# nanoporetech/medaka

Hardware: NVIDIA H100
Metric: pileup positions/sec (consensus inference) (higher is better)
Workload: dtype f32

## Files before the change

include/medaka_b200.h:

```cpp
#ifndef MEDAKA_B200_H
#define MEDAKA_B200_H

#include <stddef.h>
#include <stdint.h>

#ifdef __cplusplus
extern "C" {
#endif

#define MDK_OK 0
#define MDK_ERR_ARG -1
#define MDK_ERR_CUDA -2
#define MDK_ERR_STATE -3
#define MDK_ERR_UNSUPPORTED -4
#define MDK_ERR_NOMEM -5

#define MDK_PREC_TC 0
#define MDK_PREC_FP32 1

#define MDK_REC_AUTO 0
#define MDK_REC_ONE_TILE 1
#define MDK_REC_PINGPONG 2

#define MDK_NORM_TOTAL 0
#define MDK_NORM_FWD_REV 1
#define MDK_NORM_NONE 2

typedef struct mdk_engine mdk_engine;
typedef struct mdk_bam mdk_bam;
typedef struct mdk_bam_batch mdk_bam_batch;

typedef struct mdk_model_desc {
    int32_t num_features;
    int32_t gru_size;
    int32_t n_layers;
    int32_t bidirectional;
    int32_t num_classes;
} mdk_model_desc;

typedef struct mdk_timings {
    float h2d_ms;
    float inproj0_ms;
    float rec0_ms;
    float inproj1_ms;
    float rec1_ms;
    float head_ms;
    float d2h_ms;
    float total_ms;
    int32_t launches;
} mdk_timings;

const char *mdk_plp_bases(void);
size_t mdk_featlen(void);
size_t mdk_fwd_del(void);
size_t mdk_rev_del(void);

const char *mdk_last_error(void);
const char *mdk_version(void);
int mdk_device_count(int *count);
int mdk_device_info(int device, int *sm_arch, int *sm_count, size_t *total_mem);

int mdk_host_alloc(size_t bytes, void **out);
int mdk_host_free(void *p);
int mdk_dev_alloc(int device, size_t bytes, void **out);
int mdk_dev_free(int device, void *p);
int mdk_memcpy_h2d(int device, void *dst_dev, const void *src_host, size_t bytes);
int mdk_memcpy_d2h(int device, void *dst_host, const void *src_dev, size_t bytes);
int mdk_dev_memset(int device, void *dst_dev, int value, size_t bytes);
int mdk_device_synchronize(int device);

int mdk_engine_create(int device, const mdk_model_desc *desc, mdk_engine **out);
int mdk_engine_destroy(mdk_engine *e);
int mdk_engine_load_gru(mdk_engine *e, int layer, int direction, const float *w_ih,
                        const float *w_hh, const float *b_ih, const float *b_hh);
int mdk_engine_load_linear(mdk_engine *e, const float *w, const float *b);
// ... 94 lines not shown
                  mdk_bam_batch **out);
int64_t mdk_bam_batch_size(mdk_bam_batch *x);
int mdk_bam_batch_arrays(mdk_bam_batch *x, const int32_t **pos, const uint16_t **flag, const uint8_t **mapq,
                         const int32_t **l_seq, const uint32_t **cigar, const int64_t **cigar_off,
                         const uint8_t **seq, const int64_t **seq_off, const uint8_t **aux, const int64_t **aux_off,
                         const char **names, const int64_t **name_off);
int mdk_bam_batch_qual(mdk_bam_batch *x, const uint8_t **qual, const int64_t **qual_off);
int mdk_bam_batch_free(mdk_bam_batch *x);

int mdk_annotate(int device, int64_t n_rec, const int32_t *pos, const uint16_t *flag, const uint8_t *mapq,
                 const uint8_t *dtype, const uint32_t *cigar, const int64_t *cigar_off, const uint8_t *seq,
                 const int64_t *seq_off, const uint8_t *contig, int32_t contig_start, int32_t contig_n,
                 int32_t contig_len, int64_t n_var, const int32_t *var_pos, const int32_t *var_ref_len,
                 const int64_t *hap_off, const int64_t *allele_off, const uint8_t *alleles, int32_t pad,
                 int32_t min_mapq, int32_t dpsp, const int8_t *score, int32_t gap_open, int32_t gap_extend,
                 int64_t *dp_out, int64_t *sr_out, int64_t *ar_out, int64_t *sc_out, int64_t *stats_out,
                 float *kernel_ms);

int mdk_decode_consensus(int device, const float *probs, int64_t n, uint8_t *labels_out,
                         uint8_t *quals_out);
int mdk_decode_consensus_dev(int device, const float *probs_dev, int64_t n,
                             uint8_t *labels_out_dev, uint8_t *quals_out_dev);
int mdk_decode_consensus_f64(int device, const double *probs, int64_t n, uint8_t *labels_out,
                             uint8_t *quals_out);

int mdk_stitch_consensus(int device, const float *const *seg_probs, const int64_t *seg_rows, int64_t n_seg,
                         uint8_t *seq_out, uint8_t *qual_out, int64_t *seg_out_off);
int mdk_stitch_consensus_dev(int device, const float *probs_dev, int64_t n_rows, const int64_t *seg_base,
                             int64_t n_seg, uint8_t *seq_out_dev, uint8_t *qual_out_dev, int64_t *seg_out_off);
int mdk_stitch_labels_dev(int device, const uint8_t *labels_dev, const uint8_t *quals_dev,
                          const int64_t *seg_start, const int64_t *seg_rows, int64_t n_seg,
                          uint8_t *seq_out, uint8_t *qual_out, int64_t *seg_out_off);
int mdk_variant_join_cuts(int device, const uint8_t *const *seg_calls, const int64_t *seg_rows, int64_t n_seg,
                          int64_t *cut_out);
int mdk_decode_variants_dev(int device, const uint8_t *const *seg_calls, const float *const *seg_pred_q,
                            const float *const *seg_ref_q, const int64_t *seg_rows, int64_t n_seg,
                            const int64_t *sample_seg, int64_t n_samples, int64_t max_runs, int64_t *run_sample,
                            int64_t *run_start, int64_t *run_len, float *run_pred_q, float *run_ref_q,
                            int64_t max_run_cols, uint8_t *run_pred, float *run_col_pred_q, float *run_col_ref_q,
                            float *ref_q_out, int64_t *n_runs_out, int64_t *n_run_cols_out);

int mdk_variant_columns(int device, const int64_t *minor, const uint8_t *reference,
                        const uint8_t *prediction, uint8_t *out, int64_t len);

int mdk_decode_variants(int device, const float *probs, const int64_t *minor, const uint8_t *ref_code, int64_t n,
                        uint8_t *pred_out, uint8_t *is_var_out, float *pred_q_out, float *ref_q_out, int64_t max_runs,
                        int64_t *run_start, int64_t *run_len, float *run_pred_q, float *run_ref_q,
                        int64_t *n_runs_out);

int mdk_selftest_umma(int device, const float *A, const float *B, float *D, int N, int K,
                      int variant);

int mdk_debug_timeline(mdk_engine *e, int n_last, float *out);
int mdk_debug_read_plog(mdk_engine *e, float *out_host, int64_t n_floats);
int mdk_rl_debug_read(mdk_rl_engine *e, int which, float *out_host, int64_t n_floats);

typedef struct mdk_trainer mdk_trainer;

#define MDK_OPT_RMSPROP 0
#define MDK_OPT_ADAM 1
#define MDK_OPT_NADAM 2
#define MDK_OPT_SGD 3

typedef struct mdk_optim_desc {
    int32_t kind;
    float alpha, beta1, beta2, eps, weight_decay, momentum, dampening, momentum_decay;
    int32_t nesterov;
} mdk_optim_desc;

typedef struct mdk_train_stats {
    double loss;
    int64_t n_correct;
    int64_t n_positions;
    float grad_norm;
    int32_t skipped;
} mdk_train_stats;

int mdk_trainer_create(int device, const mdk_model_desc *desc, mdk_trainer **out);
int mdk_trainer_destroy(mdk_trainer *tr);
int mdk_trainer_load_gru(mdk_trainer *tr, int layer, int direction, const float *w_ih, const float *w_hh,
                         const float *b_ih, const float *b_hh);
int mdk_trainer_load_linear(mdk_trainer *tr, const float *w, const float *b);
int mdk_trainer_set_optimizer(mdk_trainer *tr, const mdk_optim_desc *opt);
int mdk_trainer_step(mdk_trainer *tr, const float *feats, const int32_t *labels, int64_t B, int64_t T, float lr,
                     float max_norm, mdk_train_stats *stats);
int mdk_trainer_eval(mdk_trainer *tr, const float *feats, const int32_t *labels, int64_t B, int64_t T, float *probs,
                     float *logits, mdk_train_stats *stats);
int mdk_trainer_num_params(mdk_trainer *tr, int64_t *n);
int mdk_trainer_read_params(mdk_trainer *tr, float *out_host, int64_t n);
int mdk_trainer_read_grads(mdk_trainer *tr, float *out_host, int64_t n);
int mdk_trainer_workspace_bytes(const mdk_model_desc *desc, int64_t B, int64_t T, size_t *bytes, size_t *budget);
int mdk_trainer_stage_ms(mdk_trainer *tr, float *ms);
int mdk_trainer_set_bptt_windows(mdk_trainer *tr, int nb);

typedef struct mdk_rl_trainer mdk_rl_trainer;

int mdk_rl_trainer_create(int device, int32_t lstm_size, int32_t cnn_size, int32_t use_dwells, int32_t num_classes,
                          mdk_rl_trainer **out);
int mdk_rl_trainer_destroy(mdk_rl_trainer *tr);
int mdk_rl_trainer_load(mdk_rl_trainer *tr, const char *name, const float *data, int64_t n);
int mdk_rl_trainer_set_optimizer(mdk_rl_trainer *tr, const mdk_optim_desc *opt);
int mdk_rl_trainer_step(mdk_rl_trainer *tr, const int8_t *x, const int32_t *labels, int64_t B, int64_t P, int64_t D,
                        int64_t F, float lr, float max_norm, mdk_train_stats *stats);
int mdk_rl_trainer_eval(mdk_rl_trainer *tr, const int8_t *x, const int32_t *labels, int64_t B, int64_t P, int64_t D,
                        int64_t F, float *probs, float *logits, mdk_train_stats *stats);
int mdk_rl_trainer_num_params(mdk_rl_trainer *tr, int64_t *n);
// ... 15 lines not shown
```

medaka_b200/csrc/api.cu:

```cuda
#include <algorithm>
#include <cstdlib>
#include <cstring>
#include <new>

#include "common.cuh"
#include "gru_pack.cuh"

namespace mdk {

static thread_local std::string g_last_error;

void set_error(const std::string &msg) { g_last_error = msg; }

int cuda_fail(cudaError_t err, const char *what, const char *file, int line) {
    char buf[512];
    snprintf(buf, sizeof(buf), "CUDA error %d (%s) at %s:%d: %s", (int)err, cudaGetErrorString(err), file, line, what);
    g_last_error = buf;
    if (err == cudaErrorMemoryAllocation) {
        cudaGetLastError();
        return MDK_ERR_NOMEM;
    }
    return MDK_ERR_CUDA;
}

// ... 126 lines not shown
}

static int ensure_quals(mdk_lane &ln) {
    if (ln.cap_quals >= ln.cap_io && ln.d_quals) return MDK_OK;
    dev_free(ln.d_quals);
    ln.cap_quals = 0;
    int rc;
    if ((rc = dev_alloc(&ln.d_quals, (size_t)ln.cap_io))) return rc;
    ln.cap_quals = ln.cap_io;
    return MDK_OK;
}

static int ensure_var(mdk_lane &ln) {
    if (ln.cap_var >= ln.cap_io && ln.d_ref) return MDK_OK;
    dev_free(ln.d_ref); dev_free(ln.d_calls); dev_free(ln.d_pred_q); dev_free(ln.d_ref_q);
    ln.cap_var = 0;
    int rc;
    if ((rc = dev_alloc(&ln.d_ref, (size_t)ln.cap_io))) return rc;
    if ((rc = dev_alloc(&ln.d_calls, (size_t)ln.cap_io))) return rc;
    if ((rc = dev_alloc(&ln.d_pred_q, (size_t)ln.cap_io))) return rc;
    if ((rc = dev_alloc(&ln.d_ref_q, (size_t)ln.cap_io))) return rc;
    ln.cap_var = ln.cap_io;
    return MDK_OK;
}

static int run_forward256(mdk_engine *e, mdk_ws &ws, const float *feats_dev, int64_t B, int64_t T, float *probs_dev,
                          float *logits_dev, uint8_t *labels_dev, uint8_t *quals_dev, const HeadVariant *var) {
    int rc;
    if ((rc = ensure_h1(ws, H2_256))) return rc;
    const int64_t P = B * T;
    cudaStream_t s = ws.stream, s1 = ws.l1_stream;
    const bool tc = e->precision == MDK_PREC_TC;
    const LayerWeights &l0 = e->layer[0], &l1 = e->layer[1];
    float *h0 = static_cast<float *>(ws.h0);
    MDK_CUDA(cudaStreamWaitEvent(s, ws.l1_done, 0));
    MDK_CUDA(cudaEventRecord(e->ev[1], s));
    MDK_CUDA(launch_inproj0(feats_dev, l0.w_in_packed, l0.bias_gi, ws.gi, P, e->desc.num_features,
                            T, tc ? 1 : 0, s, H256));
    MDK_CUDA(cudaEventRecord(e->ev[2], s));
    if (tc) MDK_CUDA(launch_rec256_tc(ws.gi, l0.w_hh_tm, l0.b_hn_tc, h0, B, T, s));
    else MDK_CUDA(launch_rec_fp32(ws.gi, l0.w_hh_t, l0.b_hn, h0, B, T, s, H256));
    MDK_CUDA(cudaEventRecord(e->ev[3], s));
    if (tc) MDK_CUDA(launch_gemm256_tc(h0, l1.w_in_tc, l1.bias_gi_tc, ws.gi, tiled_rows(B, T), s));
    else MDK_CUDA(launch_gemm_fp32(h0, l1.w_in_packed, l1.bias_gi, ws.gi, P, H2_256, GI256_COLS, s));
    MDK_CUDA(cudaEventRecord(e->ev[4], s));
    MDK_CUDA(cudaStreamWaitEvent(s1, e->ev[4], 0));
    if (tc) MDK_CUDA(launch_rec256_tc(ws.gi, l1.w_hh_tm, l1.b_hn_tc, ws.h1, B, T, s1));
    else MDK_CUDA(launch_rec_fp32(ws.gi, l1.w_hh_t, l1.b_hn, ws.h1, B, T, s1, H256));
    MDK_CUDA(cudaEventRecord(e->ev[5], s1));
    MDK_CUDA(cudaEventRecord(ws.l1_done, s1));
    MDK_CUDA(launch_head(ws.h1, e->lin_w, e->lin_b, B, T, tc ? 1 : 0, probs_dev, logits_dev, labels_dev, s1, quals_dev,
                         var, H2_256));
    MDK_CUDA(cudaEventRecord(e->ev[6], s1));
    e->launches += 5;
    e->last.launches = 5;
    ws.last_fused_head = false;
    ws.last_B = B; ws.last_T = T; ws.last_precision = e->precision;
    e->last_ws = (int)(&ws - e->ws);
    return MDK_OK;
}

static int run_forward(mdk_engine *e, mdk_ws &ws, const float *feats_dev, int64_t B, int64_t T, float *probs_dev,
                       float *logits_dev, uint8_t *labels_dev, uint8_t *quals_dev, const HeadVariant *var) {
    int rc;
    if ((rc = prepare_weights(e))) return rc;
    if ((rc = ensure_workspace(e, ws, B, T))) return rc;
    if (e->desc.gru_size == H256)
        return run_forward256(e, ws, feats_dev, B, T, probs_dev, logits_dev, labels_dev, quals_dev, var);
    const int64_t P = B * T;
    cudaStream_t s = ws.stream, s1 = ws.l1_stream;
    const bool tc = e->precision == MDK_PREC_TC;
    int launches = 0;
    const bool fuse_x = tc && e->layer[0].w_x_tm != nullptr;
    const int64_t tiles = (B + WT - 1) / WT;
    const int tiles_per_cta = e->rec_mode == MDK_REC_PINGPONG ? 2
                            : e->rec_mode == MDK_REC_ONE_TILE ? 1
                            : fuse_x || tiles * NDIR > (int64_t)e->sm_count ? 2 : 1;
    const bool fuse_head = tc && !e->keep_act;
    if (!fuse_head && (rc = ensure_h1(ws, H2))) return rc;
    if (!fuse_x) MDK_CUDA(cudaStreamWaitEvent(s, ws.l1_done, 0));
    MDK_CUDA(cudaEventRecord(e->ev[1], s));
    if (!fuse_x) {
        MDK_CUDA(launch_inproj0(feats_dev, e->layer[0].w_in_packed, e->layer[0].bias_gi, ws.gi, P,
                                e->desc.num_features, T, tc ? 1 : 0, s));
        launches++;
    }
    MDK_CUDA(cudaEventRecord(e->ev[2], s));
    if (tc) {
        const RecX fx{feats_dev, e->layer[0].w_x_tm, e->layer[0].bias_gi_tc, e->desc.num_features};
        MDK_CUDA(launch_rec_tc(ws.gi, fuse_x ? &fx : nullptr, e->layer[0].w_hh_tm, e->layer[0].b_hn_tc, tiles_per_cta,
                               OUT_TILES, ws.h0, nullptr, B, T, s));
    } else {
        MDK_CUDA(launch_rec_fp32(ws.gi, e->layer[0].w_hh_t, e->layer[0].b_hn, (float *)ws.h0, B, T, s));
    }
    launches++;
    if (fuse_x) MDK_CUDA(cudaStreamWaitEvent(s, ws.l1_done, 0));
    MDK_CUDA(cudaEventRecord(e->ev[3], s));
    if (tc) MDK_CUDA(launch_gemm_tc(ws.h0, e->layer[1].w_in_tc, e->layer[1].bias_gi_tc, ws.gi, tiled_rows(B, T), e->sm_count, s));
    else MDK_CUDA(launch_gemm_fp32((const float *)ws.h0, e->layer[1].w_in_packed, e->layer[1].bias_gi, ws.gi, P, H2, GI_COLS, s));
    launches++;
    MDK_CUDA(cudaEventRecord(e->ev[4], s));
    MDK_CUDA(cudaStreamWaitEvent(s1, e->ev[4], 0));
    if (tc) {
        MDK_CUDA(launch_rec_tc(ws.gi, nullptr, e->layer[1].w_hh_tm, e->layer[1].b_hn_tc, tiles_per_cta,
                               fuse_head ? OUT_LOGITS : OUT_ROWS, fuse_head ? (void *)ws.plog : ws.h1, e->lin_w, B, T, s1));
    } else {
        MDK_CUDA(launch_rec_fp32(ws.gi, e->layer[1].w_hh_t, e->layer[1].b_hn, ws.h1, B, T, s1));
    }
    launches++;
    MDK_CUDA(cudaEventRecord(e->ev[5], s1));
    MDK_CUDA(cudaEventRecord(ws.l1_done, s1));
    if (fuse_head) MDK_CUDA(launch_head_plog(ws.plog, e->lin_b, B, T, probs_dev, logits_dev, labels_dev, s1, quals_dev, var));
    else MDK_CUDA(launch_head(ws.h1, e->lin_w, e->lin_b, B, T, tc ? 1 : 0, probs_dev, logits_dev, labels_dev, s1, quals_dev,
                              var));
    launches++;
    MDK_CUDA(cudaEventRecord(e->ev[6], s1));
    e->launches += launches;
    e->last.launches = launches;
    ws.last_fused_head = fuse_head;
    ws.last_B = B; ws.last_T = T; ws.last_precision = e->precision;
    e->last_ws = (int)(&ws - e->ws);
    return MDK_OK;
}

static int acquire_lane(mdk_engine *e, int64_t P, int *out) {
    int idx;
    if (P > mdk_engine::SMALL_POS) {
        idx = e->next_big;
        e->next_big = (e->next_big + 1) % mdk_engine::BIG_LANES;
    } else {
        idx = mdk_engine::BIG_LANES + e->next_small;
        e->next_small = (e->next_small + 1) % mdk_engine::SMALL_LANES;
    }
    mdk_lane &ln = e->lane[idx];
    if (ln.busy) {
        MDK_CUDA(cudaEventSynchronize(ln.ev_out));
        ln.busy = false;
    }
    *out = idx;
    return MDK_OK;
}

struct GruCall {
    mdk_engine *e;
    const float *feats = nullptr;
    int64_t B = 0, T = 0;
    const uint8_t *ref = nullptr;

    int open(int64_t windows) {
        const int rc = acquire_lane(e, B * T, &e->open_lane);
        return rc ? rc : ensure_io(e, e->lane[e->open_lane], windows, T);
    }
    int64_t capacity(int64_t len) {
        const mdk_lane &ln = e->lane[e->open_lane];
        return std::min(ln.cap_io / len, ln.cap_feats / (len * e->desc.num_features));
    }
    int stage(int64_t first, int64_t n, int64_t at) {
        const size_t w = (size_t)T * e->desc.num_features;
        mdk_lane &ln = e->lane[e->open_lane];
        MDK_CUDA(cudaMemcpyAsync(ln.d_feats + at * w, feats + first * w, n * w * sizeof(float), cudaMemcpyDefault,
                                 e->copy_in));
        if (ref) {
            int rc;
            if ((rc = ensure_var(ln))) return rc;
            MDK_CUDA(cudaMemcpyAsync(ln.d_ref + at * T, ref + first * T, n * T, cudaMemcpyDefault, e->copy_in));
        }
        return MDK_OK;
    }
    int launch() {
// ... 362 lines not shown

static void stage_times(cudaEvent_t *ev, mdk_timings *t) {
    t->h2d_ms = ev_ms(ev[0], ev[1]);
    t->inproj0_ms = ev_ms(ev[1], ev[2]);
    t->rec0_ms = ev_ms(ev[2], ev[3]);
    t->inproj1_ms = ev_ms(ev[3], ev[4]);
    t->rec1_ms = ev_ms(ev[4], ev[5]);
    t->head_ms = ev_ms(ev[5], ev[6]);
    t->d2h_ms = ev_ms(ev[6], ev[7]);
    t->total_ms = ev_ms(ev[0], ev[7]);
}

int mdk_engine_last_timings(mdk_engine *e, mdk_timings *out) { return mdk_engine_mean_timings(e, 1, out); }

int mdk_engine_mean_timings(mdk_engine *e, int n_last, mdk_timings *out) {
    MDK_REQUIRE(e && out, MDK_ERR_ARG, "NULL argument");
    MDK_REQUIRE(n_last >= 1 && n_last <= mdk_engine::EV_RING, MDK_ERR_ARG, "mean_timings: n_last out of range");
    MDK_CUDA(cudaSetDevice(e->device));
    int rc = launch_group(e);
    if (rc) return rc;
    MDK_REQUIRE(e->fwd_count >= 1, MDK_ERR_STATE, "mean_timings: no forward recorded");
    n_last = (int)std::min<int64_t>(n_last, e->fwd_count);
    for (auto &ws : e->ws) MDK_CUDA(ws_sync(ws));
    mdk_timings acc{};
    for (int i = 0; i < n_last; ++i) {
        mdk_timings t{};
        stage_times(e->evr[(e->fwd_count - 1 - i) % mdk_engine::EV_RING], &t);
        acc.h2d_ms += t.h2d_ms; acc.inproj0_ms += t.inproj0_ms; acc.rec0_ms += t.rec0_ms;
        acc.inproj1_ms += t.inproj1_ms; acc.rec1_ms += t.rec1_ms; acc.head_ms += t.head_ms;
        acc.d2h_ms += t.d2h_ms; acc.total_ms += t.total_ms;
    }
    const float inv = 1.0f / (float)n_last;
    acc.h2d_ms *= inv; acc.inproj0_ms *= inv; acc.rec0_ms *= inv; acc.inproj1_ms *= inv; acc.rec1_ms *= inv;
    acc.head_ms *= inv; acc.d2h_ms *= inv; acc.total_ms *= inv;
    acc.launches = e->last.launches;
    *out = acc;
    return MDK_OK;
}

int mdk_debug_timeline(mdk_engine *e, int n_last, float *out) {
    MDK_REQUIRE(e && out, MDK_ERR_ARG, "NULL argument");
    MDK_CUDA(cudaSetDevice(e->device));
    int rc = launch_group(e);
    if (rc) return rc;
    MDK_REQUIRE(n_last >= 1 && n_last <= mdk_engine::EV_RING && e->fwd_count >= n_last, MDK_ERR_ARG, "timeline: bad n_last");
    for (auto &ws : e->ws) MDK_CUDA(ws_sync(ws));
    for (int i = 0; i < n_last; ++i) {
        cudaEvent_t *ev = e->evr[(e->fwd_count - n_last + i) % mdk_engine::EV_RING];
        for (int k = 0; k < 8; ++k) MDK_CUDA(cudaEventElapsedTime(out + i * 8 + k, e->ev_timer[0], ev[k]));
    }
    return MDK_OK;
}

int mdk_engine_timer_start(mdk_engine *e) {
    MDK_REQUIRE(e, MDK_ERR_ARG, "engine is NULL");
    MDK_CUDA(cudaSetDevice(e->device));
    int rc = mdk_engine_sync(e);
    if (rc) return rc;
    MDK_CUDA(cudaEventRecord(e->ev_timer[0], e->stream));
    for (int i = 0; i < mdk_engine::N_WS; ++i) {
        if (i) MDK_CUDA(cudaStreamWaitEvent(e->ws[i].stream, e->ev_timer[0], 0));
        MDK_CUDA(cudaStreamWaitEvent(e->ws[i].l1_stream, e->ev_timer[0], 0));
    }
    MDK_CUDA(cudaStreamWaitEvent(e->copy_in, e->ev_timer[0], 0));
    return MDK_OK;
}
int mdk_engine_timer_stop(mdk_engine *e, float *elapsed_ms) {
    MDK_REQUIRE(e && elapsed_ms, MDK_ERR_ARG, "NULL argument");
    MDK_CUDA(cudaSetDevice(e->device));
    int rc = launch_group(e);
    if (rc) return rc;
    for (int i = 0; i < mdk_engine::N_WS; ++i) {
        if (i) {
            MDK_CUDA(cudaEventRecord(e->ev_join, e->ws[i].stream));
            MDK_CUDA(cudaStreamWaitEvent(e->stream, e->ev_join, 0));
        }
        MDK_CUDA(cudaEventRecord(e->ev_join, e->ws[i].l1_stream));
        MDK_CUDA(cudaStreamWaitEvent(e->stream, e->ev_join, 0));
    }
    MDK_CUDA(cudaEventRecord(e->ev_join, e->copy_out.stream));
    MDK_CUDA(cudaStreamWaitEvent(e->stream, e->ev_join, 0));
    MDK_CUDA(cudaEventRecord(e->ev_timer[1], e->stream));
    MDK_CUDA(cudaEventSynchronize(e->ev_timer[1]));
    MDK_CUDA(cudaEventElapsedTime(elapsed_ms, e->ev_timer[0], e->ev_timer[1]));
    return MDK_OK;
}

int mdk_engine_read_activation(mdk_engine *e, int which, float *out_host, int64_t n_floats) {
    MDK_REQUIRE(e, MDK_ERR_ARG, "engine is NULL");
    return mdk_engine_read_activation_windows(e, which, 0, e->ws[e->last_ws].last_B, out_host, n_floats);
}

int mdk_engine_read_activation_windows(mdk_engine *e, int which, int64_t first, int64_t count, float *out_host,
                                       int64_t n_floats) {
    MDK_REQUIRE(e && out_host, MDK_ERR_ARG, "NULL argument");
    MDK_REQUIRE(which == 0 || which == 1, MDK_ERR_ARG, "read_activation: which must be 0 or 1");
    mdk_ws &ln = e->ws[e->last_ws];
    MDK_REQUIRE(ln.last_B > 0 && ln.last_T > 0, MDK_ERR_STATE, "read_activation: no forward recorded");
    MDK_REQUIRE(first >= 0 && count > 0 && first + count <= ln.last_B, MDK_ERR_ARG,
                "read_activation: windows first .. first + count - 1 must lie in the last forward's B windows");
    const int width = 2 * e->desc.gru_size;
    MDK_REQUIRE(n_floats == count * ln.last_T * width, MDK_ERR_ARG, "read_activation: size must be count*T*2*gru_size");
    MDK_REQUIRE(!(which == 1 && ln.last_fused_head), MDK_ERR_STATE,
                "read_activation(1): the last forward fused the head into layer 1 (h1 never reached HBM); call "
                "mdk_engine_keep_activations(e, 1) before the forward");
    MDK_CUDA(cudaSetDevice(e->device));
// ... 54 lines not shown
```

medaka_b200/csrc/common.cuh:

```cuda
#pragma once
#include <cuda_runtime.h>
#include <cuda_fp16.h>

#include <cstdint>
#include <cstdio>
#include <string>
#include <vector>

#include "../../include/medaka_b200.h"
#include "packing.h"

namespace mdk {

constexpr int H = 128;
constexpr int G3 = 3 * H;
constexpr int NDIR = 2;
constexpr int GI_COLS = NDIR * G3;
constexpr int H2 = NDIR * H;
constexpr int NCLS = 5;
constexpr int H256 = 256;
constexpr int G3_256 = 3 * H256;
constexpr int GI256_COLS = NDIR * G3_256;
constexpr int H2_256 = NDIR * H256;

// ... 174 lines not shown
}

struct mdk_ws {
    cudaStream_t stream = nullptr;
    cudaStream_t l1_stream = nullptr;
    cudaEvent_t l1_done = nullptr;
    int64_t cap_pos = 0;
    float *gi = nullptr;
    void *h0 = nullptr;
    float *h1 = nullptr;
    int64_t cap_h1 = 0;
    float *plog = nullptr;
    int64_t last_B = 0, last_T = 0;
    int last_precision = -1;
    bool last_fused_head = false;
};

struct mdk_lane {
    mdk_ws *ws = nullptr;
    int64_t cap_io = 0;
    int64_t cap_quals = 0;
    int64_t cap_var = 0;
    int64_t cap_feats = 0;
    float *d_feats = nullptr, *d_probs = nullptr, *d_logits = nullptr;
    uint8_t *d_labels = nullptr, *d_quals = nullptr;
    uint8_t *d_ref = nullptr, *d_calls = nullptr;
    float *d_pred_q = nullptr, *d_ref_q = nullptr;
    cudaEvent_t ev_in = nullptr, ev_out = nullptr;
    bool busy = false;
};

struct mdk_engine {
    int device = 0;
    mdk_model_desc desc{};
    int precision = MDK_PREC_TC;
    int sm_count = 132;
    int rec_mode = MDK_REC_AUTO;
    int64_t wave256 = 0;
    static constexpr int BIG_WS = 1, BIG_LANES = 4, SMALL_LANES = 14;
    static constexpr int N_LANES = BIG_LANES + SMALL_LANES, N_WS = BIG_WS + SMALL_LANES;
    static constexpr int64_t SMALL_POS = 1 << 18;
    mdk_ws ws[N_WS];
    mdk_lane lane[N_LANES];
    int next_big = 0, next_small = 0;
    mdk::Packing pk;
    int open_lane = -1;
    int last_ws = 0;
    int64_t group_windows = 0;
    cudaStream_t stream = nullptr;
    static constexpr int EV_RING = 32;
    cudaEvent_t evr[EV_RING][8] = {};
    cudaEvent_t *ev = evr[0];
    int64_t fwd_count = 0;
    cudaEvent_t ev_timer[2] = {};
    cudaEvent_t ev_join = nullptr;
    mdk::LayerWeights layer[2];
    std::vector<float> lin_w_host, lin_b_host;
    float *lin_w = nullptr, *lin_b = nullptr;
    mdk::DeviceWeights weights;
    bool keep_act = false;
    bool prepared = false;
    cudaStream_t copy_in = nullptr;
    mdk::CopyOut copy_out;
    mdk_timings last{};
    int64_t launches = 0;
};

namespace mdk {

cudaError_t launch_inproj0(const float *feats, const float *w_packed, const float *bias, float *gi,
                           int64_t P, int F, int64_t T, int tiled, cudaStream_t s, int hs = H);
enum { HEAD_PLAIN = 0, HEAD_QUALS = 1, HEAD_VARIANT = 2 };
cudaError_t launch_head(const float *h1, const float *lin_w, const float *lin_b, int64_t B, int64_t T, int tiled,
                        float *probs, float *logits, uint8_t *labels, cudaStream_t s, uint8_t *quals = nullptr,
                        const HeadVariant *var = nullptr, int width = H2);
cudaError_t launch_untile_rows(const float *src_tiled, float *dst, int64_t w0, int64_t nw, int64_t T, cudaStream_t s,
                               int width = H2);
cudaError_t launch_unpack_h0(const void *h0_tiles, float *out, int64_t w0, int64_t nw, int64_t T, cudaStream_t s);
cudaError_t launch_rec_fp32(const float *gi, const float *w_hh_t, const float *b_hn, float *h_out, int64_t B,
                            int64_t T, cudaStream_t s, int hs = H, float *save = nullptr);
cudaError_t launch_gemm_fp32(const float *A, const float *W, const float *bias, float *C, int64_t M, int K, int N,
                             cudaStream_t s);
struct RecX {
    const float *feats;
    const __half *w_x;
    const float *bias;
    int F;
};
enum { OUT_TILES = 0, OUT_ROWS = 1, OUT_LOGITS = 2 };
cudaError_t launch_rec_tc(const float *gi, const RecX *xin, const __half *w_hh_tm, const float *b_hn, int tiles_per_cta,
                          int out_kind, void *out, const float *lin_w, int64_t B, int64_t T, cudaStream_t s);
cudaError_t launch_head_plog(const float *plog, const float *lin_b, int64_t B, int64_t T, float *probs, float *logits,
                             uint8_t *labels, cudaStream_t s, uint8_t *quals = nullptr,
                             const HeadVariant *var = nullptr);
constexpr int PLOG_TS_FLOATS = NCLS * WT;
cudaError_t launch_gemm_tc(const void *x_tiles, const __half *w_in_tm, const float *bias, float *gi, int64_t P,
                           int sm_count, cudaStream_t s);
int selftest_umma(int device, const float *A, const float *B, float *D, int N, int K, int variant);
cudaError_t launch_rec256_tc(const float *gi, const __half *w_hh_tm, const float *b_hn, float *h_out, int64_t B,
                             int64_t T, cudaStream_t s);
cudaError_t rec256_max_clusters(int *clusters);
cudaError_t launch_gemm256_tc(const float *h0, const __half *w_in_tm, const float *bias, float *gi, int64_t M,
                              cudaStream_t s);
cudaError_t launch_scan_blocks(int64_t *counts, int64_t n, cudaStream_t s);
struct Records {
    const int32_t *pos;
    const uint16_t *flag;
    const uint8_t *mapq, *dtype;
    const uint32_t *cigar;
    const int64_t *cigar_off;
    const uint8_t *seq;
    const int64_t *seq_off;
};
int pileup_counts_dev(int64_t n_rec, const Records &d, int64_t n_ops, int32_t start, int32_t end, int num_dtypes,
                      int min_mapq, int64_t max_cols, uint64_t *counts, int64_t *major, int64_t *minor,
                      int64_t *n_cols_host, cudaStream_t s);

}
```

medaka_b200/csrc/gru_wg.cu:

```cuda
#include "common.cuh"
#include "ptx.cuh"
#include "rec_common.cuh"

namespace mdk {

constexpr int RW_THREADS = 256;
constexpr int RW_ABLK = (H / 8) * 64 * 16;
constexpr int RW_XBLK = 2 * 64 * 16;

template <int NT, bool FUSE_X, int OUT>
struct RwCfg {
    static constexpr int N = NT * RT_N;
    static constexpr bool HL = NT == 1;
    static constexpr int ROWS = HL ? 2 * N : N;
    static constexpr int PLANES = HL ? 1 : 2;
    static constexpr int KG = ROWS * 16 + 16;
    static_assert(KG % 16 == 0, "stmatrix rows are 16-byte aligned");
    static constexpr int HPLANE = (H / 8) * KG;
    static constexpr int XPLANE = 2 * KG;
    static constexpr int HLO = HL ? N * 16 : HPLANE;
    static constexpr int XLO = HL ? N * 16 : XPLANE;
    static constexpr int RED = (RW_THREADS / 32) * NCLS * N;
    static constexpr int wlo_off = 0;
    static constexpr int wxlo_off = wlo_off + 6 * RW_ABLK;
    static constexpr int h_off = wxlo_off + (FUSE_X ? 6 * RW_XBLK : 0);
    static constexpr int x_off = h_off + 2 * PLANES * HPLANE;
    static constexpr int red_off = x_off + (FUSE_X ? 2 * PLANES * XPLANE : 0);
    static constexpr int total = red_off + (OUT == OUT_LOGITS ? 2 * RED * 4 : 0);
    static_assert(total <= 227 * 1024, "smem budget");
};

__device__ __forceinline__ uint32_t ld_u32(const __half *p) { return *reinterpret_cast<const uint32_t *>(p); }

template <int NT, bool FUSE_X, int OUT>
__global__ void __launch_bounds__(RW_THREADS, 1)
rec_tc_kernel(const float *__restrict__ gi, RecX xin, const __half *__restrict__ w_hh, const float *__restrict__ b_hn,
              void *__restrict__ h_out, int64_t B, int64_t T, const float *__restrict__ lin_w,
              float *__restrict__ plog) {
    using L = RwCfg<NT, FUSE_X, OUT>;
    constexpr int N = L::N, NA = N / 2;
    constexpr int NACC = L::ROWS / 2;
    constexpr int NX = FUSE_X ? NACC : NA;
    using MMA = Wgmma<N>;
    using MMA_H = Wgmma<L::ROWS>;
    constexpr bool LOGITS = OUT == OUT_LOGITS;
    extern __shared__ __align__(128) uint8_t smem[];
    const int tid = threadIdx.x, wg = tid >> 7, warp = (tid >> 5) & 3, lane = tid & 31;
    const int gq = lane >> 2, cq = lane & 3;
    const int dir = blockIdx.y;
    const int64_t ntiles = (B + RT_N - 1) / RT_N;
    const int64_t wtile0 = (int64_t)blockIdx.x * NT;
    const int j0 = wg * 64 + warp * 16 + gq;
    const uint32_t sbase = smem_u32(smem);

    for (int i = tid; i < (L::total - L::h_off) / 16; i += RW_THREADS)
        reinterpret_cast<int4 *>(smem + L::h_off)[i] = make_int4(0, 0, 0, 0);
    for (int i = tid; i < 3 * H * (H / 8); i += RW_THREADS) {
        const int kg = i & 15, r = (i >> 4) & (H - 1), gate = i >> 11;
        const uint4 v = *reinterpret_cast<const uint4 *>(w_hh + ((((size_t)dir * 2 + 1) * 3 + gate) * H + r) * H + kg * 8);
        *reinterpret_cast<uint4 *>(smem + L::wlo_off + (gate * 2 + (r >> 6)) * RW_ABLK + kg * 1024 + (r & 63) * 16) = v;
    }
    if (FUSE_X) {
        for (int i = tid; i < 3 * H * 2; i += RW_THREADS) {
            const int kg = i & 1, r = (i >> 1) & (H - 1), gate = i >> 8;
            const uint4 v = *reinterpret_cast<const uint4 *>(xin.w_x + ((((size_t)dir * 2 + 1) * 3 + gate) * H + r) * 16 + kg * 8);
            *reinterpret_cast<uint4 *>(smem + L::wxlo_off + (gate * 2 + (r >> 6)) * RW_XBLK + kg * 1024 + (r & 63) * 16) = v;
        }
    }
    float wlin[2][NCLS];
    if (LOGITS) {
#pragma unroll
        for (int hb = 0; hb < 2; ++hb)
#pragma unroll
            for (int c = 0; c < NCLS; ++c) wlin[hb][c] = lin_w[c * H2 + dir * H + j0 + 8 * hb];
    }
    uint32_t whi[3][H / 16][4];
#pragma unroll
    for (int gate = 0; gate < 3; ++gate)
#pragma unroll
        for (int ks = 0; ks < H / 16; ++ks) {
            const __half *w = w_hh + ((((size_t)dir * 2) * 3 + gate) * H + j0) * H + ks * 16 + 2 * cq;
            whi[gate][ks][0] = ld_u32(w);
            whi[gate][ks][1] = ld_u32(w + 8 * H);
            whi[gate][ks][2] = ld_u32(w + 8);
            whi[gate][ks][3] = ld_u32(w + 8 * H + 8);
        }
    uint32_t wxhi[3][4];
    float bx[3][2] = {};
    if (FUSE_X) {
#pragma unroll
        for (int gate = 0; gate < 3; ++gate) {
            const __half *w = xin.w_x + ((((size_t)dir * 2) * 3 + gate) * H + j0) * 16 + 2 * cq;
// ... 214 lines not shown
        wg_hold(ar); wg_hold(az); wg_hold(an); wg_hold(axn);

#pragma unroll
        for (int k = 0; k < NA; ++k) {
            float pr = ar[k], pz = az[k], pn = an[k], px = axn[k];
            if constexpr (L::HL) {
                pr += ar[k + NA]; pz += az[k + NA]; pn += an[k + NA];
                if constexpr (FUSE_X) px += axn[k + NA];
            }
            const float a = 1.f + ex2_approx(fminf(pr, EXP_CLAMP)), b = 1.f + ex2_approx(fminf(pz, EXP_CLAMP));
            const float q = rcp_approx(a * b);
            const float r = b * q, z = a * q;
            const float en = ex2_approx(fminf(fmaf(r, pn, px), EXP_CLAMP));
            const float n = (en - 1.f) * rcp_approx(en + 1.f);
            hp[k] = fmaf(z, hp[k] - n, n);
        }
#pragma unroll
        for (int i = 0; i < N / 8; ++i) {
            uint32_t hi[2], lo[2];
#pragma unroll
            for (int hb = 0; hb < 2; ++hb) split_f16x2(hp[4 * i + 2 * hb], hp[4 * i + 2 * hb + 1], hi[hb], lo[hb]);
            stmatrix_x4_trans(hst_addr + (buf ^ 1) * L::PLANES * L::HPLANE + i * 128, hi[0], hi[1], lo[0], lo[1]);
        }
        if (FUSE_X && step + 1 < T) {
#pragma unroll
            for (int m = 0; m < NT; ++m) {
                if (xoff[m] < 0) continue;
                stage_x(buf ^ 1, m, xreg[m]);
            }
        }
        if (OUT == OUT_ROWS) {
#pragma unroll
            for (int k = 0; k < NA; ++k) {
                const int i = k >> 2, n = 8 * i + 2 * cq + (k & 1);
                const int64_t wt = wtile0 + (i >> 1);
                if (wt >= ntiles) continue;
                const int64_t orow = (wt * T + t) * RT_N + (n & 15);
                reinterpret_cast<float *>(h_out)[orow * H2 + dir * H + j0 + 8 * ((k >> 1) & 1)] = hp[k];
            }
        }
        if (FUSE_X || step + 1 < T) load_pre(dir ? t - 1 : t + 1);
        fence_proxy_async_smem();
        __syncthreads();
    }
    if (OUT == OUT_TILES) store_h0((int)(T & 1), dir ? 0 : T - 1);
    if (LOGITS) {
        if (T > 1) head_store((int)((T - 1) & 1), dir ? 1 : T - 2);
        head_partials((int)(T & 1));
        __syncthreads();
        head_store((int)(T & 1), dir ? 0 : T - 1);
    }
}

template <int NT, bool FX, int OUT>
static cudaError_t launch_rec(const float *gi, const RecX &xin, const __half *w_hh_tm, const float *b_hn, void *out,
                              const float *lin_w, int64_t B, int64_t T, cudaStream_t s) {
    auto kern = rec_tc_kernel<NT, FX, OUT>;
    constexpr int smem_bytes = RwCfg<NT, FX, OUT>::total;
    cudaError_t e = cudaFuncSetAttribute(kern, cudaFuncAttributeMaxDynamicSharedMemorySize, smem_bytes);
    if (e != cudaSuccess) return e;
    const int64_t tiles = (B + RT_N - 1) / RT_N;
    dim3 grid((unsigned)((tiles + NT - 1) / NT), NDIR);
    constexpr bool LOGITS = OUT == OUT_LOGITS;
    kern<<<grid, RW_THREADS, smem_bytes, s>>>(gi, xin, w_hh_tm, b_hn, LOGITS ? nullptr : out, B, T, lin_w,
                                              LOGITS ? static_cast<float *>(out) : nullptr);
    return cudaGetLastError();
}

template <int NT>
static cudaError_t launch_rec_nt(const float *gi, const RecX *xin, const __half *w_hh_tm, const float *b_hn, int out_kind,
                                 void *out, const float *lin_w, int64_t B, int64_t T, cudaStream_t s) {
    if (xin)
        return out_kind == OUT_TILES ? launch_rec<NT, true, OUT_TILES>(gi, *xin, w_hh_tm, b_hn, out, nullptr, B, T, s)
                                     : cudaErrorInvalidValue;
    const RecX none{nullptr, nullptr, nullptr, 0};
    switch (out_kind) {
    case OUT_TILES: return launch_rec<NT, false, OUT_TILES>(gi, none, w_hh_tm, b_hn, out, nullptr, B, T, s);
    case OUT_ROWS: return launch_rec<NT, false, OUT_ROWS>(gi, none, w_hh_tm, b_hn, out, nullptr, B, T, s);
    case OUT_LOGITS:
        return lin_w ? launch_rec<NT, false, OUT_LOGITS>(gi, none, w_hh_tm, b_hn, out, lin_w, B, T, s) : cudaErrorInvalidValue;
    }
    return cudaErrorInvalidValue;
}

cudaError_t launch_rec_tc(const float *gi, const RecX *xin, const __half *w_hh_tm, const float *b_hn, int tiles_per_cta,
                          int out_kind, void *out, const float *lin_w, int64_t B, int64_t T, cudaStream_t s) {
    if (B == 0 || T == 0) return cudaSuccess;
    switch (tiles_per_cta) {
    case 1: return launch_rec_nt<1>(gi, xin, w_hh_tm, b_hn, out_kind, out, lin_w, B, T, s);
    case 2: return launch_rec_nt<2>(gi, xin, w_hh_tm, b_hn, out_kind, out, lin_w, B, T, s);
    }
    return cudaErrorInvalidValue;
}

constexpr int GW_THREADS = 256;
constexpr int GW_QK = 8;
constexpr int GW_STAGE_PLANE = GW_QK * XT_ROWS * 16;
constexpr int GW_STAGE = 2 * GW_STAGE_PLANE;
constexpr int GW_NQ = XT_K / 8 / GW_QK;
constexpr int GW_KS = XT_K / 16;
constexpr int GW_TS = XT_ROWS / WT;
constexpr int GW_QUAD = H * 4;
constexpr int GW_QUAD_PAD = GW_QUAD + 16;
constexpr int GW_OUT_OFF = GW_NQ * GW_STAGE;
constexpr int GW_BAR_OFF = GW_OUT_OFF + GW_TS * 4 * GW_QUAD_PAD * 4;
constexpr int GW_SMEM = GW_BAR_OFF + 2 * GW_NQ * 8;
static_assert(GW_SMEM <= 227 * 1024, "smem budget");
static_assert(GW_TS * 4 == 32, "one bulk store per lane of warp 0");

__global__ void __launch_bounds__(GW_THREADS, 1)
gemm_tc_kernel(const uint8_t *__restrict__ x_tiles, const __half *__restrict__ w_in_tm, const float *__restrict__ bias,
               float *__restrict__ gi, int64_t P, int64_t ntiles) {
    extern __shared__ __align__(128) uint8_t smem[];
    uint64_t *full = reinterpret_cast<uint64_t *>(smem + GW_BAR_OFF), *empty = full + GW_NQ;
    float *stg = reinterpret_cast<float *>(smem + GW_OUT_OFF);
    const int tid = threadIdx.x, wg = tid >> 7, warp = (tid >> 5) & 3, lane = tid & 31;
    const int gq = lane >> 2, cq = lane & 3;
    const int blk = blockIdx.x;
    const int j0 = wg * 64 + warp * 16 + gq;
    const uint32_t sbase = smem_u32(smem);
    const int64_t my_tiles = blockIdx.y < ntiles ? (ntiles - 1 - blockIdx.y) / gridDim.y + 1 : 0;
    auto issue = [&](int64_t n, int q) {
        const uint8_t *src = x_tiles + (blockIdx.y + n * gridDim.y) * (int64_t)XT_TILE_BYTES + q * GW_STAGE_PLANE;
        mbar_arrive_expect_tx(&full[q], GW_STAGE);
        bulk_g2s(smem + q * GW_STAGE, src, GW_STAGE_PLANE, &full[q]);
        bulk_g2s(smem + q * GW_STAGE + GW_STAGE_PLANE, src + XT_PLANE_BYTES, GW_STAGE_PLANE, &full[q]);
    };
    if (tid == 0) {
        for (int q = 0; q < GW_NQ; ++q) {
            mbar_init(&full[q], 1);
            mbar_init(&empty[q], GW_THREADS / 32);
        }
        fence_mbar_init();
        if (my_tiles > 0)
            for (int q = 0; q < GW_NQ; ++q) issue(0, q);
    }
    uint32_t wa[2][GW_KS][4];
#pragma unroll
    for (int p = 0; p < 2; ++p)
#pragma unroll
        for (int ks = 0; ks < GW_KS; ++ks) {
            const __half *w = w_in_tm + (((size_t)blk * 2 + p) * H + j0) * H2 + ks * 16 + 2 * cq;
            wa[p][ks][0] = ld_u32(w);
// ... 149 lines not shown
```

medaka_b200/csrc/packing.h:

```cpp
#pragma once
#include <algorithm>
#include <cstdint>
#include <vector>

namespace mdk {

struct Packing {
    struct Piece {
        float *probs, *logits;
        uint8_t *labels;
        int64_t first, n;
        uint8_t *quals;
        const uint8_t *ref;
        float *pred_q, *ref_q;
    };
    std::vector<Piece> pieces;
    int64_t windows = 0, len = 0;
    bool open = false;
    int64_t serial = -1;
    int64_t launched = -1;
    static constexpr int TICKET_RING = 4096;
    int64_t ticket_group[TICKET_RING] = {};
    int64_t tickets = 0;

    template <class Eng>
    int launch(Eng &&eng) {
        if (!open) return 0;
        open = false;
        if (pieces.empty()) return 0;
        const int rc = eng.launch();
        if (!rc) launched = serial;
        return rc;
    }

    template <class Eng>
    int enqueue(Eng &&eng, int64_t B, int64_t L, float *probs, float *logits, uint8_t *labels, int64_t gmax,
                int64_t *ticket, uint8_t *quals = nullptr, const uint8_t *ref = nullptr, float *pred_q = nullptr,
                float *ref_q = nullptr) {
        int rc;
        if (open && len != L && (rc = launch(eng))) return rc;
        for (int64_t done = 0; done < B;) {
            if (!open) {
                if ((rc = eng.open(std::min(B - done, gmax)))) return rc;
                pieces.clear();
                windows = 0; len = L;
                open = true;
                serial++;
            }
            int64_t room = std::min(gmax, eng.capacity(L)) - windows;
            if (windows == 0) room = std::max<int64_t>(room, 1);
            if (room < 1) {
                if ((rc = launch(eng))) return rc;
                continue;
            }
            const int64_t n = std::min(room, B - done);
            if ((rc = eng.stage(done, n, windows))) return rc;
            pieces.push_back(Piece{probs, logits, labels, done, n, quals, ref, pred_q, ref_q});
            windows += n;
            done += n;
            if (done == B && ticket) {
                ticket_group[tickets % TICKET_RING] = serial;
                *ticket = tickets++;
            }
            if (n == room && (rc = launch(eng))) return rc;
        }
        return 0;
    }

    template <class Eng>
    int settle(Eng &&eng, int64_t ticket, int64_t *group) {
        *group = ticket_group[std::max(ticket, tickets - TICKET_RING) % TICKET_RING];
        return open && *group == serial ? launch(eng) : 0;
    }
};

}
```

medaka_b200/models.py:

```python
import collections
import inspect
import logging
import warnings

import numpy as np

from medaka_b200 import libmedaka as _lm

ForwardOutput = collections.namedtuple("ForwardOutput", ["probs", "logits", "labels"])

_PRECISIONS = {"tc": 0, "half": 0, "fp32": 1, "full": 1}


def _as_f32(x):
    if hasattr(x, "detach"):
        x = x.detach().cpu().numpy()
    return np.ascontiguousarray(x, dtype=np.float32)


class PinnedArray(object):

    def __init__(self, shape, dtype):
        lib = _lm.load()
        self.shape = tuple(int(s) for s in shape)
# ... 216 lines not shown
            raise ValueError("ref_bytes must be [B, T] = [{}, {}], got {}".format(B, T, tuple(ref_bytes.shape)))
        lib, ffi = _lm.lib, _lm.ffi

        def ptr(x, ctype):
            if isinstance(x, int):
                return ffi.cast(ctype, x)
            if hasattr(x, "data_ptr"):
                if not x.is_contiguous():
                    raise ValueError("tensors must be contiguous")
                return ffi.cast(ctype, x.data_ptr())
            return ffi.cast(ctype, ffi.from_buffer(x))

        ticket = ffi.new("int64_t *")
        _lm.check(lib.mdk_engine_submit_variant_decoded(
            self._engine, ptr(feats, "const float *"), B, T, ptr(ref_bytes, "const uint8_t *"),
            ptr(calls_out, "uint8_t *"), ptr(pred_q_out, "float *"), ptr(ref_q_out, "float *"), ticket))
        self._last_shape = (B, T)
        return int(ticket[0])

    def sync(self):
        _lm.check(_lm.lib.mdk_engine_sync(self._engine))

    def wait(self, ticket):
        _lm.check(_lm.lib.mdk_engine_wait(self._engine, ticket))

    def predict_async(self, batch, slots=2):
        x = _as_f32(self.get_model_input_features(batch))
        B, T, F = x.shape
        slot = getattr(self, "_async_n", 0) % max(int(slots), 1)
        self._async_n = getattr(self, "_async_n", 0) + 1
        xin = self.pinned("afeats%d" % slot, (B, T, F), np.float32)
        np.copyto(xin, x)
        probs = self.pinned("aprobs%d" % slot, (B, T, 5), np.float32)
        labels = self.pinned("alabels%d" % slot, (B, T), np.uint8)
        ticket = self.submit_arrays(xin, probs, labels)
        return AsyncResult(self, lambda: self.wait(ticket), probs, labels)

    def lookahead(self, batch_size, window_len=None):
        pref = self.preferred_batch_size()
        if window_len is not None and batch_size * window_len <= (1 << 18):
            return 14
        return int(max(2, min(64, 4 * ((pref + batch_size - 1) // max(batch_size, 1)) + 1)))

    def reserve(self, windows, window_len):
        _lm.check(_lm.lib.mdk_engine_reserve(self._engine, int(windows), int(window_len)))

    def flush(self):
        _lm.check(_lm.lib.mdk_engine_flush(self._engine))

    def set_rec_mode(self, mode):
        code = {"auto": _lm.lib.MDK_REC_AUTO, "one": _lm.lib.MDK_REC_ONE_TILE, "pp": _lm.lib.MDK_REC_PINGPONG}[mode]
        _lm.check(_lm.lib.mdk_engine_set_rec_mode(self._engine, code))

    def set_group_windows(self, windows):
        _lm.check(_lm.lib.mdk_engine_set_group_windows(self._engine, int(windows)))

    def forward(self, x):
        import torch
        out = self.forward_arrays(_as_f32(x), want_logits=not self.normalise, want_labels=False)
        return torch.from_numpy(out.probs if self.normalise else out.logits)

    def predict_on_batch(self, batch):
        import torch
        out = self.forward_arrays(_as_f32(self.get_model_input_features(batch)), want_logits=False,
                                  want_labels=True)
        self.last_labels = out.labels
        return torch.from_numpy(out.probs)

    def last_timings(self):
        t = _lm.ffi.new("mdk_timings *")
        _lm.check(_lm.lib.mdk_engine_last_timings(self._engine, t))
        return {k: getattr(t, k) for k in ("h2d_ms", "inproj0_ms", "rec0_ms", "inproj1_ms", "rec1_ms",
                                             "head_ms", "d2h_ms", "total_ms", "launches")}

    def read_activation(self, which, first=0, count=None):
        t = self.last_timings()
        del t
        shape = self._last_shape
        count = shape[0] - first if count is None else count
        out = np.empty((count, shape[1], 2 * self.gru_size), dtype=np.float32)
        _lm.check(_lm.lib.mdk_engine_read_activation_windows(
            self._engine, which, first, count, _lm.ffi.cast("float *", _lm.ffi.from_buffer(out)), out.size))
        return out

    def read_plog(self):
        t = self.last_timings()
        del t
        B, T = self._last_shape
        out = np.empty((2, (B + 15) // 16, T, 5, 16), dtype=np.float32)
        _lm.check(_lm.lib.mdk_debug_read_plog(self._engine, _lm.ffi.cast("float *", _lm.ffi.from_buffer(out)), out.size))
        return out

    def launch_count(self):
        return int(_lm.lib.mdk_engine_launch_count(self._engine))

    def keep_activations(self, keep=True):
        _lm.check(_lm.lib.mdk_engine_keep_activations(self._engine, 1 if keep else 0))

    def preferred_batch_size(self):
        return int(_lm.lib.mdk_engine_preferred_windows(self._engine))

    @property
    def engine(self):
        return self._engine

    def close(self):
# ... 29 lines not shown
```

Measured before the change: 184.2 million.

## Add ordered one-tile recurrence variant and pick tiles per layer

Splits the one-tile-per-CTA recurrence into two variants: the existing hi/lo merged-operand form and a new ordered form that uses two planes. With fused input projection and a single wave, each GRU layer now picks its variant separately, using whether the previous layer-1 ran two tiles and whether the packed batch was full. Before, fused-x always used two tiles per CTA. The goal is to cut per-step latency for small batches, at the cost of more template instantiations, cross-call state and a new introspection API.

```diff
diff --git a/include/medaka_b200.h b/include/medaka_b200.h
--- a/include/medaka_b200.h
+++ b/include/medaka_b200.h
@@ -21,6 +21,11 @@
 #define MDK_REC_AUTO 0
 #define MDK_REC_ONE_TILE 1
 #define MDK_REC_PINGPONG 2
+
+#define MDK_TILES_NONE 0
+#define MDK_TILES_ONE_MERGED 1
+#define MDK_TILES_ONE_ORDERED 2
+#define MDK_TILES_TWO 3
 
 #define MDK_NORM_TOTAL 0
 #define MDK_NORM_FWD_REV 1
@@ -221,6 +226,7 @@
                       int variant);
 
 int mdk_debug_timeline(mdk_engine *e, int n_last, float *out);
+int mdk_engine_rec_tiles(mdk_engine *e, int n_last, int *out);
 int mdk_debug_read_plog(mdk_engine *e, float *out_host, int64_t n_floats);
 int mdk_rl_debug_read(mdk_rl_engine *e, int which, float *out_host, int64_t n_floats);
 
diff --git a/medaka_b200/csrc/api.cu b/medaka_b200/csrc/api.cu
--- a/medaka_b200/csrc/api.cu
+++ b/medaka_b200/csrc/api.cu
@@ -202,6 +202,9 @@
     MDK_CUDA(launch_head(ws.h1, e->lin_w, e->lin_b, B, T, tc ? 1 : 0, probs_dev, logits_dev, labels_dev, s1, quals_dev,
                          var, H2_256));
     MDK_CUDA(cudaEventRecord(e->ev[6], s1));
+    int *rec_tiles = e->rec_tiles[(e->fwd_count - 1) % mdk_engine::EV_RING];
+    rec_tiles[0] = rec_tiles[1] = MDK_TILES_NONE;
+    e->l1_two = false;
     e->launches += 5;
     e->last.launches = 5;
     ws.last_fused_head = false;
@@ -223,9 +226,15 @@
     int launches = 0;
     const bool fuse_x = tc && e->layer[0].w_x_tm != nullptr;
     const int64_t tiles = (B + WT - 1) / WT;
-    const int tiles_per_cta = e->rec_mode == MDK_REC_PINGPONG ? 2
-                            : e->rec_mode == MDK_REC_ONE_TILE ? 1
-                            : fuse_x || tiles * NDIR > (int64_t)e->sm_count ? 2 : 1;
+    const bool one_wave = tiles * NDIR <= (int64_t)e->sm_count;
+    RecTiles rt[2];
+    if (e->rec_mode == MDK_REC_PINGPONG) rt[0] = rt[1] = REC_TWO;
+    else if (e->rec_mode == MDK_REC_ONE_TILE) rt[0] = rt[1] = REC_ONE_MERGED;
+    else if (!fuse_x) rt[0] = rt[1] = one_wave ? REC_ONE_MERGED : REC_TWO;
+    else {
+        rt[0] = e->l1_two || !one_wave ? REC_TWO : REC_ONE_ORDERED;
+        rt[1] = e->pk.full || !one_wave ? REC_TWO : REC_ONE_ORDERED;
+    }
     const bool fuse_head = tc && !e->keep_act;
     if (!fuse_head && (rc = ensure_h1(ws, H2))) return rc;
     if (!fuse_x) MDK_CUDA(cudaStreamWaitEvent(s, ws.l1_done, 0));
@@ -238,7 +247,7 @@
     MDK_CUDA(cudaEventRecord(e->ev[2], s));
     if (tc) {
         const RecX fx{feats_dev, e->layer[0].w_x_tm, e->layer[0].bias_gi_tc, e->desc.num_features};
-        MDK_CUDA(launch_rec_tc(ws.gi, fuse_x ? &fx : nullptr, e->layer[0].w_hh_tm, e->layer[0].b_hn_tc, tiles_per_cta,
+        MDK_CUDA(launch_rec_tc(ws.gi, fuse_x ? &fx : nullptr, e->layer[0].w_hh_tm, e->layer[0].b_hn_tc, rt[0],
                                OUT_TILES, ws.h0, nullptr, B, T, s));
     } else {
         MDK_CUDA(launch_rec_fp32(ws.gi, e->layer[0].w_hh_t, e->layer[0].b_hn, (float *)ws.h0, B, T, s));
@@ -252,7 +261,7 @@
     MDK_CUDA(cudaEventRecord(e->ev[4], s));
     MDK_CUDA(cudaStreamWaitEvent(s1, e->ev[4], 0));
     if (tc) {
-        MDK_CUDA(launch_rec_tc(ws.gi, nullptr, e->layer[1].w_hh_tm, e->layer[1].b_hn_tc, tiles_per_cta,
+        MDK_CUDA(launch_rec_tc(ws.gi, nullptr, e->layer[1].w_hh_tm, e->layer[1].b_hn_tc, rt[1],
                                fuse_head ? OUT_LOGITS : OUT_ROWS, fuse_head ? (void *)ws.plog : ws.h1, e->lin_w, B, T, s1));
     } else {
         MDK_CUDA(launch_rec_fp32(ws.gi, e->layer[1].w_hh_t, e->layer[1].b_hn, ws.h1, B, T, s1));
@@ -265,6 +274,10 @@
                               var));
     launches++;
     MDK_CUDA(cudaEventRecord(e->ev[6], s1));
+    int *rec_tiles = e->rec_tiles[(e->fwd_count - 1) % mdk_engine::EV_RING];
+    rec_tiles[0] = tc ? rt[0] : MDK_TILES_NONE;
+    rec_tiles[1] = tc ? rt[1] : MDK_TILES_NONE;
+    e->l1_two = tc && rt[1] == REC_TWO;
     e->launches += launches;
     e->last.launches = launches;
     ws.last_fused_head = fuse_head;
@@ -733,6 +746,21 @@
     return MDK_OK;
 }
 
+int mdk_engine_rec_tiles(mdk_engine *e, int n_last, int *out) {
+    MDK_REQUIRE(e && out, MDK_ERR_ARG, "NULL argument");
+    MDK_CUDA(cudaSetDevice(e->device));
+    int rc = launch_group(e);
+    if (rc) return rc;
+    MDK_REQUIRE(n_last >= 1 && n_last <= mdk_engine::EV_RING && e->fwd_count >= n_last, MDK_ERR_ARG,
+                "rec_tiles: bad n_last");
+    for (int i = 0; i < n_last; ++i) {
+        const int *t = e->rec_tiles[(e->fwd_count - n_last + i) % mdk_engine::EV_RING];
+        out[2 * i] = t[0];
+        out[2 * i + 1] = t[1];
+    }
+    return MDK_OK;
+}
+
 int mdk_engine_timer_start(mdk_engine *e) {
     MDK_REQUIRE(e, MDK_ERR_ARG, "engine is NULL");
     MDK_CUDA(cudaSetDevice(e->device));
diff --git a/medaka_b200/csrc/common.cuh b/medaka_b200/csrc/common.cuh
--- a/medaka_b200/csrc/common.cuh
+++ b/medaka_b200/csrc/common.cuh
@@ -250,6 +250,8 @@
     cudaEvent_t evr[EV_RING][8] = {};
     cudaEvent_t *ev = evr[0];
     int64_t fwd_count = 0;
+    int rec_tiles[EV_RING][2] = {};
+    bool l1_two = false;
     cudaEvent_t ev_timer[2] = {};
     cudaEvent_t ev_join = nullptr;
     mdk::LayerWeights layer[2];
@@ -286,7 +288,8 @@
     int F;
 };
 enum { OUT_TILES = 0, OUT_ROWS = 1, OUT_LOGITS = 2 };
-cudaError_t launch_rec_tc(const float *gi, const RecX *xin, const __half *w_hh_tm, const float *b_hn, int tiles_per_cta,
+enum RecTiles { REC_ONE_MERGED = MDK_TILES_ONE_MERGED, REC_ONE_ORDERED = MDK_TILES_ONE_ORDERED, REC_TWO = MDK_TILES_TWO };
+cudaError_t launch_rec_tc(const float *gi, const RecX *xin, const __half *w_hh_tm, const float *b_hn, RecTiles tiles,
                           int out_kind, void *out, const float *lin_w, int64_t B, int64_t T, cudaStream_t s);
 cudaError_t launch_head_plog(const float *plog, const float *lin_b, int64_t B, int64_t T, float *probs, float *logits,
                              uint8_t *labels, cudaStream_t s, uint8_t *quals = nullptr,
diff --git a/medaka_b200/csrc/gru_wg.cu b/medaka_b200/csrc/gru_wg.cu
--- a/medaka_b200/csrc/gru_wg.cu
+++ b/medaka_b200/csrc/gru_wg.cu
@@ -8,10 +8,11 @@
 constexpr int RW_ABLK = (H / 8) * 64 * 16;
 constexpr int RW_XBLK = 2 * 64 * 16;
 
-template <int NT, bool FUSE_X, int OUT>
+template <int NT, bool HL_, bool FUSE_X, int OUT>
 struct RwCfg {
+    static_assert(!HL_ || NT == 1, "the hi/lo operand of 2N rows exists at one tile per CTA only");
     static constexpr int N = NT * RT_N;
-    static constexpr bool HL = NT == 1;
+    static constexpr bool HL = HL_;
     static constexpr int ROWS = HL ? 2 * N : N;
     static constexpr int PLANES = HL ? 1 : 2;
     static constexpr int KG = ROWS * 16 + 16;
@@ -32,12 +33,12 @@
 
 __device__ __forceinline__ uint32_t ld_u32(const __half *p) { return *reinterpret_cast<const uint32_t *>(p); }
 
-template <int NT, bool FUSE_X, int OUT>
+template <int NT, bool HL, bool FUSE_X, int OUT>
 __global__ void __launch_bounds__(RW_THREADS, 1)
 rec_tc_kernel(const float *__restrict__ gi, RecX xin, const __half *__restrict__ w_hh, const float *__restrict__ b_hn,
               void *__restrict__ h_out, int64_t B, int64_t T, const float *__restrict__ lin_w,
               float *__restrict__ plog) {
-    using L = RwCfg<NT, FUSE_X, OUT>;
+    using L = RwCfg<NT, HL, FUSE_X, OUT>;
     constexpr int N = L::N, NA = N / 2;
     constexpr int NACC = L::ROWS / 2;
     constexpr int NX = FUSE_X ? NACC : NA;
@@ -358,11 +359,11 @@
     }
 }
 
-template <int NT, bool FX, int OUT>
+template <int NT, bool HL, bool FX, int OUT>
 static cudaError_t launch_rec(const float *gi, const RecX &xin, const __half *w_hh_tm, const float *b_hn, void *out,
                               const float *lin_w, int64_t B, int64_t T, cudaStream_t s) {
-    auto kern = rec_tc_kernel<NT, FX, OUT>;
-    constexpr int smem_bytes = RwCfg<NT, FX, OUT>::total;
+    auto kern = rec_tc_kernel<NT, HL, FX, OUT>;
+    constexpr int smem_bytes = RwCfg<NT, HL, FX, OUT>::total;
     cudaError_t e = cudaFuncSetAttribute(kern, cudaFuncAttributeMaxDynamicSharedMemorySize, smem_bytes);
     if (e != cudaSuccess) return e;
     const int64_t tiles = (B + RT_N - 1) / RT_N;
@@ -373,28 +374,32 @@
     return cudaGetLastError();
 }
 
-template <int NT>
+template <int NT, bool HL>
 static cudaError_t launch_rec_nt(const float *gi, const RecX *xin, const __half *w_hh_tm, const float *b_hn, int out_kind,
                                  void *out, const float *lin_w, int64_t B, int64_t T, cudaStream_t s) {
     if (xin)
-        return out_kind == OUT_TILES ? launch_rec<NT, true, OUT_TILES>(gi, *xin, w_hh_tm, b_hn, out, nullptr, B, T, s)
+        return out_kind == OUT_TILES ? launch_rec<NT, HL, true, OUT_TILES>(gi, *xin, w_hh_tm, b_hn, out, nullptr, B, T, s)
                                      : cudaErrorInvalidValue;
     const RecX none{nullptr, nullptr, nullptr, 0};
     switch (out_kind) {
-    case OUT_TILES: return launch_rec<NT, false, OUT_TILES>(gi, none, w_hh_tm, b_hn, out, nullptr, B, T, s);
-    case OUT_ROWS: return launch_rec<NT, false, OUT_ROWS>(gi, none, w_hh_tm, b_hn, out, nullptr, B, T, s);
+    case OUT_TILES:
+        if constexpr (NT == 1 && !HL) return cudaErrorInvalidValue;
+        else return launch_rec<NT, HL, false, OUT_TILES>(gi, none, w_hh_tm, b_hn, out, nullptr, B, T, s);
+    case OUT_ROWS: return launch_rec<NT, HL, false, OUT_ROWS>(gi, none, w_hh_tm, b_hn, out, nullptr, B, T, s);
     case OUT_LOGITS:
-        return lin_w ? launch_rec<NT, false, OUT_LOGITS>(gi, none, w_hh_tm, b_hn, out, lin_w, B, T, s) : cudaErrorInvalidValue;
+        return lin_w ? launch_rec<NT, HL, false, OUT_LOGITS>(gi, none, w_hh_tm, b_hn, out, lin_w, B, T, s)
+                     : cudaErrorInvalidValue;
     }
     return cudaErrorInvalidValue;
 }
 
-cudaError_t launch_rec_tc(const float *gi, const RecX *xin, const __half *w_hh_tm, const float *b_hn, int tiles_per_cta,
+cudaError_t launch_rec_tc(const float *gi, const RecX *xin, const __half *w_hh_tm, const float *b_hn, RecTiles tiles,
                           int out_kind, void *out, const float *lin_w, int64_t B, int64_t T, cudaStream_t s) {
     if (B == 0 || T == 0) return cudaSuccess;
-    switch (tiles_per_cta) {
-    case 1: return launch_rec_nt<1>(gi, xin, w_hh_tm, b_hn, out_kind, out, lin_w, B, T, s);
-    case 2: return launch_rec_nt<2>(gi, xin, w_hh_tm, b_hn, out_kind, out, lin_w, B, T, s);
+    switch (tiles) {
+    case REC_ONE_MERGED: return launch_rec_nt<1, true>(gi, xin, w_hh_tm, b_hn, out_kind, out, lin_w, B, T, s);
+    case REC_ONE_ORDERED: return launch_rec_nt<1, false>(gi, xin, w_hh_tm, b_hn, out_kind, out, lin_w, B, T, s);
+    case REC_TWO: return launch_rec_nt<2, false>(gi, xin, w_hh_tm, b_hn, out_kind, out, lin_w, B, T, s);
     }
     return cudaErrorInvalidValue;
 }
diff --git a/medaka_b200/csrc/packing.h b/medaka_b200/csrc/packing.h
--- a/medaka_b200/csrc/packing.h
+++ b/medaka_b200/csrc/packing.h
@@ -19,15 +19,17 @@
     bool open = false;
     int64_t serial = -1;
     int64_t launched = -1;
+    bool full = false;
     static constexpr int TICKET_RING = 4096;
     int64_t ticket_group[TICKET_RING] = {};
     int64_t tickets = 0;
 
     template <class Eng>
-    int launch(Eng &&eng) {
+    int launch(Eng &&eng, bool is_full = false) {
         if (!open) return 0;
         open = false;
         if (pieces.empty()) return 0;
+        full = is_full;
         const int rc = eng.launch();
         if (!rc) launched = serial;
         return rc;
@@ -50,7 +52,7 @@
             int64_t room = std::min(gmax, eng.capacity(L)) - windows;
             if (windows == 0) room = std::max<int64_t>(room, 1);
             if (room < 1) {
-                if ((rc = launch(eng))) return rc;
+                if ((rc = launch(eng, windows >= gmax))) return rc;
                 continue;
             }
             const int64_t n = std::min(room, B - done);
@@ -62,7 +64,7 @@
                 ticket_group[tickets % TICKET_RING] = serial;
                 *ticket = tickets++;
             }
-            if (n == room && (rc = launch(eng))) return rc;
+            if (n == room && (rc = launch(eng, windows >= gmax))) return rc;
         }
         return 0;
     }
diff --git a/medaka_b200/models.py b/medaka_b200/models.py
--- a/medaka_b200/models.py
+++ b/medaka_b200/models.py
@@ -292,6 +292,13 @@
         code = {"auto": _lm.lib.MDK_REC_AUTO, "one": _lm.lib.MDK_REC_ONE_TILE, "pp": _lm.lib.MDK_REC_PINGPONG}[mode]
         _lm.check(_lm.lib.mdk_engine_set_rec_mode(self._engine, code))
 
+    def rec_tiles(self, n_last=1):
+        out = _lm.ffi.new("int[]", 2 * n_last)
+        _lm.check(_lm.lib.mdk_engine_rec_tiles(self._engine, int(n_last), out))
+        names = {_lm.lib.MDK_TILES_NONE: None, _lm.lib.MDK_TILES_ONE_MERGED: "one-merged",
+                 _lm.lib.MDK_TILES_ONE_ORDERED: "one", _lm.lib.MDK_TILES_TWO: "two"}
+        return [(names[out[2 * i]], names[out[2 * i + 1]]) for i in range(n_last)]
+
     def set_group_windows(self, windows):
         _lm.check(_lm.lib.mdk_engine_set_group_windows(self._engine, int(windows)))
 
```

After: 188.9 million, median of 6. +2.5%, better.
